# MarkTakken/kf2vecFSW

Measured on AMD Instinct MI355X. Metric: Gbases/s k-mer→.kf build at k=7; achieved HBM GB/s vs gfx950 peak, higher is better.
Workload: dtype u32

## Files before the change

### include/kf2vec_gpu.h

```cpp
#ifndef KF2VEC_GPU_H
#define KF2VEC_GPU_H

#include <stddef.h>
#include <stdint.h>

#ifdef __cplusplus
extern "C" {
#endif

#define KF_ABI_VERSION 1

#define KF_OK 0
#define KF_EINVAL (-1)
#define KF_EHIP (-2)
#define KF_ERANGE (-3)
#define KF_EFORMAT (-4)

#define KF_MIN_K 2
#define KF_MAX_K 12
#define KF_SPARSE_MAX_K 31

#define KF_ACCUMULATE 1u

#define KF_FMT_AUTO 0
// ... 19 lines not shown
int kf_index_fasta(const uint8_t* d_bytes, const uint64_t* d_goff, int32_t n_genomes,
                   uint64_t batch_bytes, uint64_t* d_excl, uint64_t cap_pairs,
                   uint64_t* d_n_pairs, uint32_t* d_scratch, uint64_t scratch_words, void* stream);

uint64_t kf_index_fastq_scratch_bytes(uint64_t batch_bytes, int32_t n_genomes, uint64_t cap_lines);
int kf_index_fastq(const uint8_t* d_bytes, const uint64_t* d_goff, int32_t n_genomes,
                   uint64_t batch_bytes, uint64_t* d_excl, uint64_t cap_pairs, uint64_t cap_lines,
                   uint64_t* d_n, uint32_t* d_status, void* d_scratch, uint64_t scratch_bytes,
                   void* stream);

int kf_count_batch(const uint8_t* d_bytes, const uint64_t* d_goff, int32_t n_genomes,
                   const uint64_t* d_excl, uint64_t n_excl,
                   const uint32_t* d_code2col, const uint32_t* d_col2rep, int k,
                   uint32_t* d_counts, uint64_t* d_totals, uint32_t flags, void* stream);

int kf_rows_accumulate(const uint32_t* d_src, const uint64_t* d_src_totals, int32_t n_src,
                       const int32_t* d_seg, int32_t n_dst, uint64_t nbins,
                       uint32_t* d_dst, uint64_t* d_dst_totals, uint32_t* d_status,
                       uint32_t flags, void* stream);

int kf_workspace_reserve(int k, int32_t max_genomes);

int kf_count_launch_info(int k, int* grid, int* block, int* lds_bytes);

uint64_t kf_sparse_workspace_bytes(int k, uint64_t batch_bytes, int32_t n_genomes);
int kf_sparse_count(const uint8_t* d_bytes, const uint64_t* d_goff, int32_t n_genomes,
                    uint64_t batch_bytes, const uint64_t* d_excl, uint64_t n_excl, int k,
                    void* d_work, uint64_t work_bytes, uint64_t* d_keys, uint32_t* d_counts,
                    uint64_t* d_nuniq, void* stream);

int kf_kmers_tile_rows(void);
int kf_kmers_rows(const uint64_t* d_keys, const void* d_counts, int count_bytes,
                  const uint64_t* d_src0, const uint64_t* d_n, const uint64_t* d_dst0,
                  const float* d_denom, int32_t n_seg, int k, uint64_t row_lo, uint64_t row_hi,
                  float* d_out, uint32_t* d_status, void* stream);

int      kf_sparse_merge_tile(void);
uint64_t kf_sparse_merge_scratch_bytes(uint64_t n_a, uint64_t n_b);
int kf_sparse_merge(const uint64_t* d_keys_a, const void* d_counts_a, int count_bytes_a, uint64_t n_a,
                    const uint64_t* d_keys_b, const void* d_counts_b, int count_bytes_b, uint64_t n_b,
                    uint64_t* d_keys_out, uint64_t* d_counts_out, uint64_t* d_n_out,
                    uint32_t* d_status, void* d_scratch, uint64_t scratch_bytes, void* stream);

uint64_t kf_chunk_features_scratch_bytes(int32_t n_samples);
int kf_chunk_features(const void* d_counts, int count_bytes, uint64_t n_rows, uint64_t nbins,
                      const uint64_t* d_lo, const uint64_t* d_n, int32_t n_samples,
// ... 59 lines not shown
```

### kf2vecfsw_amd/_native.py

```python
from __future__ import annotations

import ctypes
import os

_HERE = os.path.dirname(os.path.abspath(__file__))
LIB_PATH = os.environ.get("KF2VEC_GPU_LIB") or os.path.join(_HERE, "libkf2vec_gpu.so")

KF_OK = 0
KF_EINVAL = -1
KF_EHIP = -2
KF_ERANGE = -3
KF_EFORMAT = -4
KF_MIN_K = 2
KF_MAX_K = 12
KF_SPARSE_MAX_K = 31
KF_ACCUMULATE = 1
KF_FMT_AUTO, KF_FMT_FASTA, KF_FMT_FASTQ = 0, 1, 2

_u64, _u32, _i32, _i64, _int = ctypes.c_uint64, ctypes.c_uint32, ctypes.c_int32, ctypes.c_int64, ctypes.c_int
_vp, _cp = ctypes.c_void_p, ctypes.c_char_p
_P64 = ctypes.POINTER(ctypes.c_uint64)
_PI = ctypes.POINTER(ctypes.c_int)
SIGNATURES = {
    "kf_abi_version": (_int, []),
    "kf_last_error": (_cp, []),
    "kf_num_bins": (_u64, [_int]),
    "kf_tables": (_int, [_int, _vp, _vp, _P64]),
    "kf_vocab_text": (_int, [_int, _vp, _u64, _P64]),
    "kf_index_records": (_int, [_vp, _u64, _int, _u64, _vp, _u64, _P64, _PI]),
    "kf_count_batch": (_int, [_vp, _vp, _i32, _vp, _u64, _vp, _vp, _int, _vp, _vp, _u32, _vp]),
    "kf_rows_accumulate": (_int, [_vp, _vp, _i32, _vp, _i32, _u64, _vp, _vp, _vp, _u32, _vp]),
    "kf_count_launch_info": (_int, [_int, _PI, _PI, _PI]),
    "kf_workspace_release": (_int, []),
    "kf_workspace_reserve": (_int, [_int, _i32]),
    "kf_build_id": (_cp, []),
    "kf_stream_probe": (_int, [_vp, _u64, _vp, _vp]),
    "kf_synth_fasta": (_int, [_vp, _vp, _i32, _i64, _i64, _u64, _u64, _int, _u64, _vp]),
    "kf_synth_genome_bytes": (_u64, [_i64, _u64, _int, _u64]),
    "kf_synth_header_len": (_u64, [_i64]),
    "kf_format_kf": (_int, [_cp, _vp, _u64, _int, _int, _vp, _u64, _P64]),
    "kf_write_kf_files": (_int, [_cp, ctypes.POINTER(_cp), _i32, _vp, _u64, _int, _int, _int]),
    "kf_write_kf_rows": (_int, [_cp, ctypes.POINTER(_cp), _i32, _vp, _u64, _int, _int, _int]),
    "kf_write_kf_segments": (_int, [_i32, ctypes.POINTER(_cp), _vp, _vp, ctypes.POINTER(_cp), ctypes.POINTER(_cp),
                                    _vp, _vp, _u32, _vp, _u64, _int, _int, _int]),
    "kf_write_kf_segments16": (_int, [_i32, ctypes.POINTER(_cp), _vp, _vp, ctypes.POINTER(_cp), ctypes.POINTER(_cp),
                                      _vp, _vp, _u32, _vp, _u64, _int, _int, _int]),
    "kf_chunk_compact": (_int, [_vp, _u64, _vp, _i32, _vp, _vp, _vp, _u64, _vp]),
    "kf_chunk_gather": (_int, [_vp, _vp, _i32, _u32, _vp, _vp]),
    "kf_index_fasta": (_int, [_vp, _vp, _i32, _u64, _vp, _u64, _vp, _vp, _u64, _vp]),
    "kf_index_fastq_scratch_bytes": (_u64, [_u64, _i32, _u64]),
    "kf_index_fastq": (_int, [_vp, _vp, _i32, _u64, _vp, _u64, _u64, _vp, _vp, _vp, _u64, _vp]),
    "kf_read_files":(_int, [ctypes.POINTER(_cp), _i32, _vp, _vp, _vp, _u64, _int]),
    "kf_sparse_workspace_bytes": (_u64, [_int, _u64, _i32]),
    "kf_sparse_count": (_int, [_vp, _vp, _i32, _u64, _vp, _u64, _int, _vp, _u64, _vp, _vp, _vp, _vp]),
    "kf_kmers_tile_rows": (_int, []),
# ... 6 lines not shown
                                 _vp]),
    "kf_parse_kf_scratch_bytes": (_u64, [_u64, _i32, _u64]),
    "kf_parse_kf_rows": (_int, [_vp, _vp, _i32, _u64, _u64, _u64, _vp, _vp, _vp, _vp, _u64, _vp]),
}


class NativeError(RuntimeError):
    pass


_lib = None


def lib() -> ctypes.CDLL:
    global _lib
    if _lib is None:
        if not os.path.exists(LIB_PATH):
            raise NativeError(f"{LIB_PATH} not found: build it with `python -m kf2vecfsw_amd.build`")
        import torch
        try:
            L = ctypes.CDLL(LIB_PATH)
        except OSError as e:
            raise NativeError(f"cannot load {LIB_PATH}: {e}") from e
        for name, (res, args) in SIGNATURES.items():
            fn = getattr(L, name)
            fn.restype = res
            fn.argtypes = args
        if L.kf_abi_version() != 1:
            raise NativeError("libkf2vec_gpu ABI version mismatch")
        bid = L.kf_build_id().decode()
        if "+" not in bid and os.environ.get("KF2VEC_ALLOW_FOREIGN_LIB") != "1":
            from .build import source_id
            if bid != source_id():
                raise NativeError(f"{LIB_PATH} was built from other sources (build id {bid}, sources "
                                  f"{source_id()}): rebuild with `python -m kf2vecfsw_amd.build`")
        _lib = L
    return _lib


def build_id() -> str:
    return lib().kf_build_id().decode()


def check(rc: int, what: str = "") -> None:
    if rc != KF_OK:
        msg = lib().kf_last_error().decode(errors="replace")
        raise NativeError(f"{what or 'kf2vec_gpu'} failed ({rc}): {msg}")
```

### kf2vecfsw_amd/csrc/kf_bucket.hip

```cpp
#include <hip/hip_runtime.h>
#include <stdint.h>
#include <stdlib.h>

#include <algorithm>
#include <cstdio>
#include <mutex>
#include <vector>

#include "kf_front.h"
#include "kf_internal.h"

namespace kf {


constexpr int kBkWaves = 16;
constexpr int kBkBits = 15;
constexpr uint64_t kPieceMax = (8ull << 20) - (64ull << 10);
constexpr uint32_t kBkLagShift = 3;
constexpr uint32_t kBkSlots = 2;
constexpr uint32_t kBkRoundWeights = 0x060B1114;
constexpr int kBkGroupWindows = 4;
constexpr bool bk_pre2(int K) { return K <= 10; }
constexpr uint32_t bk_rl(int K) { return K == 10 ? 4 : 0; }

// ... 880 lines not shown
}

}

extern "C" int kf_workspace_release(void) {
    int dev = 0;
    if (hipGetDevice(&dev) != hipSuccess) return kf_fail(KF_EHIP, "hipGetDevice failed");
    if (dev < 0 || dev >= 64) return kf_fail(KF_EINVAL, "device index out of range");
    std::lock_guard<std::mutex> lk(g_mu);
    DevState& d = g_dev[dev];
    if (hipDeviceSynchronize() != hipSuccess) return kf_fail(KF_EHIP, "hipDeviceSynchronize failed");
    for (int k = 0; k <= KF_MAX_K; ++k) {
        if (d.col_idx[k]) (void)hipFree(d.col_idx[k]);
        if (d.bcol[k]) (void)hipFree(d.bcol[k]);
        d.col_idx[k] = nullptr;
        d.bcol[k] = nullptr;
    }
    if (d.scratch) (void)hipFree(d.scratch);
    if (d.pstart) (void)hipFree(d.pstart);
    d.scratch = nullptr;
    d.scratch_bytes = 0;
    d.pstart = nullptr;
    d.pstart_n = 0;
    return KF_OK;
}
```

### kf2vecfsw_amd/csrc/kf_count.hip

```cpp
#include <hip/hip_runtime.h>
#include <stdint.h>
#include <stdlib.h>

#include <mutex>

#include "kf_front.h"
#include "kf_internal.h"

namespace kf {

constexpr int kBlock = 1024;
constexpr uint32_t kWaveWeights = 20u | 17u << 8 | 11u << 16 | 6u << 24;
constexpr int kXRing = 2;

__device__ __forceinline__ void wg_span(const CountArgs& A, uint64_t& lo, uint64_t& hi) {
    const uint64_t base = A.goff[0];
    const uint64_t total = A.goff[A.n_genomes] - base;
    const uint64_t G = gridDim.x, b = blockIdx.x;
    lo = base + ((total / G * b + (total % G) * b / G) & ~(uint64_t)15);
    hi = (b + 1 == G) ? base + total : base + ((total / G * (b + 1) + (total % G) * (b + 1) / G) & ~(uint64_t)15);
}

template <int K>
struct XL {
    static constexpr uint32_t P = K >= 8 ? (1u << 17) : (2u << (2 * (K + 1)));
    static constexpr uint32_t S = K >= 8 ? (1u << 15) : (2u << (2 * K));
    static constexpr uint32_t bytes = P + S;
};
constexpr int kXChunk = 3 * kChunk;
static_assert((uint32_t)kXChunk == kLattice, "wave ranges are split on the iteration lattice (split_at_lattice)");
constexpr uint32_t kLatticeMaxIters = 2560;
constexpr uint32_t kHot7 = 0xC000C000u, kStep7 = 0x4000u;
constexpr uint32_t kHot8 = 0xE000E000u, kStep8 = 0x2000u;
constexpr uint32_t kHot6 = 0x80008000u, kStep6 = 0x8000u;
template <int K>
constexpr uint32_t x_hot() { return K >= 8 ? kHot8 : (K == 7 ? kHot7 : kHot6); }
template <int K>
constexpr uint32_t x_step() { return K >= 8 ? kStep8 : (K == 7 ? kStep7 : kStep6); }

__device__ __forceinline__ uint32_t k9_code_of(uint32_t i) { return ((i >> 9) << 10) | (i & 0x1FFu); }

__device__ __forceinline__ uint32_t half_one(uint32_t i) { return 1u << ((i & 1u) << 4); }

template <int B>
__device__ __forceinline__ uint32_t shl1_byte(uint32_t h, uint32_t one) {
    uint32_t r;
    if constexpr (B == 0)
        asm("v_lshlrev_b32_sdwa %0, %1, %2 dst_sel:DWORD dst_unused:UNUSED_PAD src0_sel:BYTE_0 src1_sel:DWORD"
            : "=v"(r) : "v"(h), "v"(one));
    else if constexpr (B == 1)
        asm("v_lshlrev_b32_sdwa %0, %1, %2 dst_sel:DWORD dst_unused:UNUSED_PAD src0_sel:BYTE_1 src1_sel:DWORD"
// ... 302 lines not shown
    if constexpr (K == 9) {
        drained |= k9b_region<false>(wlo, whi, R, A, gcounts);
        lane_total += (uint32_t)__builtin_popcount(R);
        return win.next;
    }
    const uint32_t wv[4] = {wlo, __builtin_amdgcn_alignbit(whi, wlo, 8), __builtin_amdgcn_alignbit(whi, wlo, 16),
                            __builtin_amdgcn_alignbit(whi, wlo, 24)};
    uint32_t o = 0;
#pragma unroll
    for (int r = 0; r < 16; ++r) {
        const int fo = (2 * r) & ~7;
        const uint32_t y = __builtin_amdgcn_ubfe(wv[fo >> 3], 2 * r - fo, 2 * K);
        o |= lds_add_rtn((K == 8 ? 0u : XL<K>::P) + ((y >> 1) << 2), ((R >> r) & 1u) * half_one(y));
    }
    if (__builtin_amdgcn_ballot_w64((o & HOT) != 0) != 0) {
        x_scan_drain<K>(A.code2col, gcounts, lane);
        drained = 1;
    }
    lane_total += (uint32_t)__builtin_popcount(R);
    return win.next;
}

template <int K>
__device__ __forceinline__ uint32_t x_range(const CountArgs& A, int32_t g, uint64_t glo, uint64_t ghi, uint64_t lo,
                                            uint64_t hi, int lane, uint64_t& iv_hint, uint32_t& drained) {
    if (lo >= hi) return 0;
    uint32_t* gcounts = A.counts + (uint64_t)g * A.nbins;
    Range rg;
    rg.init(glo, ghi, lo, hi);
    const uint32_t lim_r = min(rg.end_r, rg.nch * (uint32_t)kChunk);
    auto load = [&](uint32_t r) {
        return xc_load(A.bytes, rg.c0, r, lim_r, lane);
    };
    static_assert(kXRing == 2, "two-deep register ring");
    XBlock buf[K == 9 ? 1 : kXRing];
    XBlock b0, b1;
    if constexpr (K == 9) {
        b0 = load(0);
        b1 = load(kXChunk);
    } else {
#pragma unroll
        for (int j = 0; j < kXRing; ++j) buf[j] = load(j * kXChunk);
    }
    const uint32_t nx = (rg.nch + 2) / 3;
    rg.warm16<K>(A, lane, iv_hint);
    __builtin_amdgcn_s_setprio(0);
    uint32_t carry = rg.carry;
    uint32_t rel = 0;
    const ChunkMask m = rg.mask();
    uint32_t lane_total = 0;
// ... 71 lines not shown
__device__ __forceinline__ void pair_f_sums_small(const uint32_t* hist, int tid,
                                                  uint32_t (&F)[((1u << (2 * K)) + kBlock - 1) / kBlock]) {
    constexpr uint32_t NY = 1u << (2 * K), NM = (NY + kBlock - 1) / kBlock;
#pragma unroll
    for (uint32_t m = 0; m < NM; ++m) {
        const uint32_t y = (uint32_t)tid + kBlock * m;
        F[m] = 0;
        if (y < NY) {
            const uint32_t sh = (y & 1u) << 4;
            uint32_t f = u16sum2(hist[2 * y]) + u16sum2(hist[2 * y + 1]);
#pragma unroll
            for (uint32_t a = 0; a < 4; ++a) f += (hist[a * (NY / 2) + (y >> 1)] >> sh) & 0xFFFFu;
            f += (hist[XL<K>::P / 4 + (y >> 1)] >> sh) & 0xFFFFu;
            F[m] = f;
        }
    }
}

__device__ __forceinline__ void lds_zero(uint32_t* hist, uint32_t lo4, uint32_t hi4, int tid) {
    uint4* h4 = (uint4*)hist;
    for (uint32_t i = lo4 + (uint32_t)tid; i < hi4; i += kBlock) h4[i] = make_uint4(0u, 0u, 0u, 0u);
}

template <int K>
__global__ void __launch_bounds__(kBlock) __attribute__((amdgpu_waves_per_eu(4, 4))) k1x_kernel(CountArgs A) {
    static_assert(K >= 2 && K <= 9, "K1x serves k = 2 .. 9 (k = 9: K9b byte counters)");
    extern __shared__ __attribute__((aligned(16))) uint32_t hist[];
    const int tid = threadIdx.x;
    const int lane = tid & (kWave - 1);
    const int wave = __builtin_amdgcn_readfirstlane(tid >> 6);
    {
        uint4* h4 = (uint4*)hist;
        for (uint32_t i = tid; i < XL<K>::bytes / 16; i += kBlock) h4[i] = make_uint4(0u, 0u, 0u, 0u);
    }
    __syncthreads();
    if ((uint32_t)(uintptr_t)(lds_u32*)hist != 0u) __builtin_trap();
    uint64_t span_lo, span_hi;
    wg_span(A, span_lo, span_hi);
    if (span_lo >= span_hi) return;
    int32_t g = (int32_t)wave_upper_bound((uint64_t)A.n_genomes, span_lo, lane,
                                          [&](uint64_t i) { return A.goff[i + 1]; });
    const uint32_t fr_lo = wave_frac((uint32_t)wave, kWaveWeights), fr_hi = wave_frac((uint32_t)wave + 1, kWaveWeights);
    uint64_t g_lo = A.goff[g], g_hi = A.goff[g + 1];
    uint64_t iv_hint = 0;
    for (; g < A.n_genomes; ++g) {
        __builtin_amdgcn_s_setprio(3);
        const uint64_t glo = g_lo, ghi = g_hi;
        g_lo = g_hi;
        g_hi = A.goff[min(g + 2, A.n_genomes)];
        if (glo >= span_hi) break;
        const uint64_t plo = max(glo, span_lo), phi = min(ghi, span_hi);
        if (phi <= plo) continue;
        const uint32_t nit = lattice_iters(plo, phi);
        const bool lat = nit <= kLatticeMaxIters;
        const uint64_t lo = split_at_lattice(plo, phi, nit, lat, fr_lo), hi = split_at_lattice(plo, phi, nit, lat, fr_hi);
        uint32_t drained = 0;
        unsigned long long s = x_range<K>(A, g, glo, ghi, lo, hi, lane, iv_hint, drained);
        uint32_t* gc = A.counts + (uint64_t)g * A.nbins;
        const bool whole = plo == glo && phi == ghi && !(A.flags & KF_ACCUMULATE);
        if constexpr (K == 9) {
            lds_barrier();
            if (lane == 0) hist[XL<K>::P / 4 + wave] = drained;
            lds_barrier();
            const uint4* fl = (const uint4*)(hist + XL<K>::P / 4);
            const uint4 f0 = fl[0], f1 = fl[1], f2 = fl[2], f3 = fl[3];
            const bool any_fix = (f0.x | f0.y | f0.z | f0.w | f1.x | f1.y | f1.z | f1.w | f2.x | f2.y | f2.z |
                                  f2.w | f3.x | f3.y | f3.z | f3.w) != 0;
            const uint8_t* hb = (const uint8_t*)hist;
            for (uint32_t c0 = (uint32_t)tid; c0 < (1u << 17); c0 += 4 * kBlock) {
                uint32_t rep[4];
#pragma unroll
                for (int j = 0; j < 4; ++j) rep[j] = A.col2rep[c0 + j * kBlock];
#pragma unroll
                for (int j = 0; j < 4; ++j) {
                    const uint32_t c = (rep[j] & 0x200u) ? kf_revcomp<9>(rep[j]) : rep[j];
                    const uint32_t v = hb[((c >> 1) & 0x1FE00u) | (c & 0x1FFu)];
                    if (whole && !any_fix)
                        __builtin_nontemporal_store(v, gc + c0 + j * kBlock);
                    else if (v)
                        __hip_atomic_fetch_add(gc + c0 + j * kBlock, v, __ATOMIC_RELAXED, __HIP_MEMORY_SCOPE_AGENT);
                }
            }
            lds_barrier();
            uint4* h4 = (uint4*)hist;
            for (uint32_t i = tid; i < XL<K>::bytes / 16; i += kBlock) h4[i] = make_uint4(0u, 0u, 0u, 0u);
        } else if constexpr (K == 8) {
            lds_barrier();
            if (lane == 0) hist[XL<K>::P / 4 + wave] = drained;
            lds_barrier();
            const uint4* fl = (const uint4*)(hist + XL<K>::P / 4);
            const uint4 f0 = fl[0], f1 = fl[1], f2 = fl[2], f3 = fl[3];
            const bool any_drain = (f0.x | f0.y | f0.z | f0.w | f1.x | f1.y | f1.z | f1.w | f2.x | f2.y | f2.z |
                                    f2.w | f3.x | f3.y | f3.z | f3.w) != 0;
            for (uint32_t col = tid; col < A.nbins; col += kBlock) {
                const uint32_t y = A.col2rep[col], rc = kf_revcomp<8>(y);
                uint32_t v = (hist[y >> 1] >> ((y & 1u) << 4)) & 0xFFFFu;
                if (rc != y) v += (hist[rc >> 1] >> ((rc & 1u) << 4)) & 0xFFFFu;
                if (whole && !any_drain)
                    gc[col] = v;
                else if (v)
                    __hip_atomic_fetch_add(gc + col, v, __ATOMIC_RELAXED, __HIP_MEMORY_SCOPE_AGENT);
            }
            lds_barrier();
            uint4* h4 = (uint4*)hist;
            for (uint32_t i = tid; i < XL<K>::bytes / 16; i += kBlock) h4[i] = make_uint4(0u, 0u, 0u, 0u);
        } else if constexpr (K <= 6) {
            constexpr uint32_t NY = 1u << (2 * K), NM = (NY + kBlock - 1) / kBlock;
            constexpr uint32_t NCOL = (NY + (K % 2 == 0 ? (1u << K) : 0u)) / 2, NC = (NCOL + kBlock - 1) / kBlock;
            constexpr uint32_t ZF = (NY + 16) / 4;
            static_assert(ZF <= XL<K>::bytes / 16, "F and the flags lie inside the table");
            uint32_t rep[NC];
#pragma unroll
            for (uint32_t c = 0; c < NC; ++c) {
                const uint32_t col = (uint32_t)tid + c * kBlock;
                rep[c] = col < NCOL ? A.col2rep[col] : 0u;
            }
            lds_barrier();
            uint32_t F[NM];
            pair_f_sums_small<K>(hist, tid, F);
            lds_barrier();
#pragma unroll
            for (uint32_t m = 0; m < NM; ++m) {
                const uint32_t y = (uint32_t)tid + kBlock * m;
                if (y < NY) hist[f_swz(y)] = F[m];
            }
            if (lane == 0) hist[NY + wave] = drained;
            lds_zero(hist, ZF, XL<K>::bytes / 16, tid);
            lds_barrier();
            const uint4* fl = (const uint4*)(hist + NY);
            const uint4 f0 = fl[0], f1 = fl[1], f2 = fl[2], f3 = fl[3];
            const bool any_drain = (f0.x | f0.y | f0.z | f0.w | f1.x | f1.y | f1.z | f1.w | f2.x | f2.y | f2.z | f2.w |
                                    f3.x | f3.y | f3.z | f3.w) != 0;
            uint32_t cv[NC];
#pragma unroll
            for (uint32_t c = 0; c < NC; ++c) {
                const uint32_t y = rep[c], rc = kf_revcomp<K>(y);
                cv[c] = hist[f_swz(y)] + (rc != y ? hist[f_swz(rc)] : 0u);
            }
            lds_barrier();
            lds_zero(hist, 0, ZF, tid);
#pragma unroll
            for (uint32_t c = 0; c < NC; ++c) {
                const uint32_t col = (uint32_t)tid + c * kBlock;
                if (col >= NCOL) continue;
                if (whole && !any_drain)
                    __builtin_nontemporal_store(cv[c], gc + col);
                else if (cv[c])
                    __hip_atomic_fetch_add(gc + col, cv[c], __ATOMIC_RELAXED, __HIP_MEMORY_SCOPE_AGENT);
            }
        } else {
            uint32_t rep[8];
            if (whole) {
                const uint4 r0 = *(const uint4*)(A.col2rep + 4 * tid), r1 = *(const uint4*)(A.col2rep + 4096 + 4 * tid);
                rep[0] = r0.x, rep[1] = r0.y, rep[2] = r0.z, rep[3] = r0.w;
                rep[4] = r1.x, rep[5] = r1.y, rep[6] = r1.z, rep[7] = r1.w;
            } else {
#pragma unroll
                for (int c = 0; c < 8; ++c) rep[c] = A.col2rep[tid + c * kBlock];
            }
            lds_barrier();
            uint32_t F[16];
            pair_f_sums(hist, tid, F);
#pragma unroll
            for (int i = 0; i < 8; ++i) {
                const uint32_t v = hist[XL<K>::P / 4 + i * 1024 + tid];
                F[2 * i] += v & 0xFFFFu;
                F[2 * i + 1] += v >> 16;
            }
            lds_barrier();
#pragma unroll
            for (int i = 0; i < 8; ++i) *(uint2*)(hist + f_swz(i * 2048 + 2 * tid)) = make_uint2(F[2 * i], F[2 * i + 1]);
            if (lane == 0) hist[16384 + wave] = drained;
            constexpr uint32_t ZF = (16384 + 16) / 4;
            lds_zero(hist, ZF, XL<K>::bytes / 16, tid);
            lds_barrier();
            const uint4* fl = (const uint4*)(hist + 16384);
            const uint4 f0 = fl[0], f1 = fl[1], f2 = fl[2], f3 = fl[3];
            const bool any_drain = (f0.x | f0.y | f0.z | f0.w | f1.x | f1.y | f1.z | f1.w | f2.x | f2.y | f2.z | f2.w |
                                    f3.x | f3.y | f3.z | f3.w) != 0;
            uint32_t cv[8];
#pragma unroll
            for (int c = 0; c < 8; ++c) {
                const uint32_t y = rep[c], rc = kf_revcomp<7>(y);
                cv[c] = hist[f_swz(y)] + hist[f_swz(rc)];
            }
            lds_barrier();
            lds_zero(hist, 0, ZF, tid);
            if (whole && !any_drain) {
                typedef unsigned int v4u_t __attribute__((ext_vector_type(4)));
                __builtin_nontemporal_store(v4u_t{cv[0], cv[1], cv[2], cv[3]}, (v4u_t*)(gc + 4 * tid));
                __builtin_nontemporal_store(v4u_t{cv[4], cv[5], cv[6], cv[7]}, (v4u_t*)(gc + 4096 + 4 * tid));
            } else {
#pragma unroll
                for (int c = 0; c < 8; ++c) {
                    const uint32_t col = whole ? (c >> 2) * 4096 + 4 * tid + (c & 3) : tid + c * kBlock;
                    if (cv[c]) __hip_atomic_fetch_add(gc + col, cv[c], __ATOMIC_RELAXED, __HIP_MEMORY_SCOPE_AGENT);
                }
            }
        }
        s = wave_sum(s);
        if (lane == 0 && s) atomicAdd(A.totals + g, s);
        lds_barrier();
    }
}

__device__ __forceinline__ uint64_t splitmix64(uint64_t x) {
    x += 0x9E3779B97F4A7C15ull;
    x = (x ^ (x >> 30)) * 0xBF58476D1CE4E5B9ull;
    x = (x ^ (x >> 27)) * 0x94D049BB133111EBull;
    return x ^ (x >> 31);
}

__device__ __forceinline__ bool in_nrun(uint64_t key, uint64_t i, uint64_t n_period) {
    if (!n_period) return false;
    uint64_t b = i >> 12;
    for (int d = 0; d < 2; ++d) {
        if (d == 1) {
            if (b == 0) break;
            b -= 1;
        }
        const uint64_t h = splitmix64((key ^ 0xA5A5A5A5A5A5A5A5ull) + b);
        if (h % n_period) continue;
        const uint64_t st = (b << 12) + ((h >> 16) % 4096), ln = 1 + ((h >> 32) % 100);
        if (i >= st && i < st + ln) return true;
// ... 124 lines not shown
int launch_info(int k, int* grid, int* block, int* lds) {
    int dev = 0;
    if (hipGetDevice(&dev) != hipSuccess) return kf_fail(KF_EHIP, "hipGetDevice failed");
    if (dev < 0 || dev >= 64) return kf_fail(KF_EINVAL, "device index out of range");
    const int l = lds_bytes_for(k);
    std::lock_guard<std::mutex> lk(g_grid_mu);
    int& gr = g_grid[k][dev];
    if (!gr) {
        void* fn = kernel_for(k);
        if (hipFuncSetAttribute(fn, hipFuncAttributeMaxDynamicSharedMemorySize, l) != hipSuccess)
            return kf_fail(KF_EHIP, "hipFuncSetAttribute(MaxDynamicSharedMemorySize) failed");
        int per_cu = 0, cus = 0;
        if (hipOccupancyMaxActiveBlocksPerMultiprocessor(&per_cu, fn, kBlock, l) != hipSuccess)
            return kf_fail(KF_EHIP, "hipOccupancyMaxActiveBlocksPerMultiprocessor failed");
        if (hipDeviceGetAttribute(&cus, hipDeviceAttributeMultiprocessorCount, dev) != hipSuccess)
            return kf_fail(KF_EHIP, "hipDeviceGetAttribute(MultiprocessorCount) failed");
        gr = (per_cu < 1 ? 1 : per_cu) * (cus > 0 ? cus : 1);
    }
    *grid = gr;
    *block = kBlock;
    *lds = l;
    return KF_OK;
}
}

extern "C" int kf_count_launch_info(int k, int* grid, int* block, int* lds_bytes) {
    if (k < KF_MIN_K || k > KF_MAX_K) return kf_fail(KF_EINVAL, "k out of range [2, 12]");
    if (!grid || !block || !lds_bytes) return kf_fail(KF_EINVAL, "null output pointer");
    if (k >= 10) return bucket_launch_info(k, grid, block, lds_bytes);
    return launch_info(k, grid, block, lds_bytes);
}

extern "C" int kf_workspace_reserve(int k, int32_t max_genomes) {
    if (k < KF_MIN_K || k > KF_MAX_K) return kf_fail(KF_EINVAL, "k out of range [2, 12]");
    if (max_genomes < 0) return kf_fail(KF_EINVAL, "max_genomes < 0");
    if (k >= 10) return bucket_reserve(k, max_genomes);
    int grid = 0, block = 0, lds = 0;
    return launch_info(k, &grid, &block, &lds);
}

extern "C" int kf_count_batch(const uint8_t* d_bytes, const uint64_t* d_goff, int32_t n_genomes,
                              const uint64_t* d_excl, uint64_t n_excl, const uint32_t* d_code2col,
                              const uint32_t* d_col2rep, int k, uint32_t* d_counts, uint64_t* d_totals,
                              uint32_t flags, void* stream) {
    if (k < KF_MIN_K || k > KF_MAX_K) return kf_fail(KF_EINVAL, "k out of range [2, 12]");
    if (n_genomes < 0) return kf_fail(KF_EINVAL, "n_genomes < 0");
    if (n_genomes == 0) return KF_OK;
    if (!d_bytes || !d_goff || !d_counts || !d_totals || !d_code2col || !d_col2rep)
        return kf_fail(KF_EINVAL, "null device pointer");
    if (n_excl && !d_excl) return kf_fail(KF_EINVAL, "d_excl is null but n_excl > 0");
    if (((uintptr_t)d_bytes) & 15) return kf_fail(KF_EINVAL, "d_bytes must be 16-byte aligned");
    const uint64_t nb = kf_num_bins(k);
    hipStream_t s = (hipStream_t)stream;
    const bool bucket = k >= 10;
    if (!(flags & KF_ACCUMULATE)) {
        if ((!bucket && hipMemsetAsync(d_counts, 0, (size_t)n_genomes * nb * sizeof(uint32_t), s) != hipSuccess) ||
            hipMemsetAsync(d_totals, 0, (size_t)n_genomes * sizeof(uint64_t), s) != hipSuccess)
            return kf_fail(KF_EHIP, "hipMemsetAsync failed");
    }
    CountArgs A;
    A.bytes = d_bytes;
    A.goff = d_goff;
    A.excl = d_excl;
    A.n_excl = n_excl;
    A.code2col = d_code2col;
    A.col2rep = d_col2rep;
    A.counts = d_counts;
    A.totals = (unsigned long long*)d_totals;
    A.nbins = (uint32_t)nb;
    A.n_genomes = n_genomes;
    A.flags = flags;
    if (bucket) return bucket_launch(A, k, flags, s);
    int grid = 0, block = 0, lds = 0;
    const int rc = launch_info(k, &grid, &block, &lds);
    if (rc) return rc;

    void* args[] = {&A};
    if (hipLaunchKernel(kernel_for(k), dim3(grid), dim3(block), args, (size_t)lds, s) != hipSuccess)
        return kf_fail(KF_EHIP, "count kernel launch failed: %s", hipGetErrorString(hipGetLastError()));
    return KF_OK;
}

extern "C" int kf_stream_probe(const uint8_t* d_bytes, uint64_t n, uint32_t* d_out, void* stream) {
    if (!d_bytes || !d_out) return kf_fail(KF_EINVAL, "null device pointer");
    if (((uintptr_t)d_bytes) & 15) return kf_fail(KF_EINVAL, "d_bytes must be 16-byte aligned");
    if (n == 0) return KF_OK;
    int dev = 0, cus = 0;
    if (hipGetDevice(&dev) != hipSuccess ||
        hipDeviceGetAttribute(&cus, hipDeviceAttributeMultiprocessorCount, dev) != hipSuccess)
        return kf_fail(KF_EHIP, "device query failed");
    hipLaunchKernelGGL(stream_probe_kernel, dim3(2 * (cus > 0 ? cus : 1)), dim3(1024), 0, (hipStream_t)stream, d_bytes,
                       n, d_out);
    if (hipGetLastError() != hipSuccess) return kf_fail(KF_EHIP, "stream probe launch failed");
    return KF_OK;
}

extern "C" int kf_synth_fasta(uint8_t* d_bytes, const uint64_t* d_goff, int32_t n_genomes, int64_t g0,
                              int64_t g_stride, uint64_t seed0, uint64_t seq_len, int width, uint64_t n_period,
                              void* stream) {
// ... 11 lines not shown
```

### kf2vecfsw_amd/csrc/kf_front.h

```cpp
#pragma once
#include <hip/hip_runtime.h>
#include <stdint.h>

#include "kf_scan.h"

namespace kf {

constexpr int kWave = 64;
constexpr int kChunk = 1024;

struct CountArgs {
    const uint8_t* bytes;
    const uint64_t* goff;
    const uint64_t* excl;
    uint64_t n_excl;
    const uint32_t* code2col;
    const uint32_t* col2rep;
    uint32_t* counts;
    unsigned long long* totals;
    uint32_t nbins;
    int32_t n_genomes;
    uint32_t flags;
};

// ... 419 lines not shown
    }
    const uint64_t W = ((uint64_t)t_codes(ctx) << (2 * ne)) | (uint64_t)C;
    Windows w;
    w.wlo = (uint32_t)W;
    w.whi = (uint32_t)(W >> 32);
    const uint32_t ctxlen = min(t_n(ctx), (uint32_t)(K - 1));
    const uint32_t E = (((1u << ctxlen) - 1u) << ne) | V;
    w.R = run_mask<K>(E) & ((1u << ne) - 1u);
    if (MASKED) w.R &= EN;
    const uint32_t incl = tail_pack(w.wlo & TM, (uint32_t)__builtin_ctz(~E), 31u);
    w.next = (uint32_t)__builtin_amdgcn_readlane((int)incl, kWave - 1);
    return w;
}

__device__ __forceinline__ unsigned long long wave_sum(unsigned long long v) {
#pragma unroll
    for (int d = 32; d >= 1; d >>= 1) v += __shfl_xor(v, d, kWave);
    return v;
}

int bucket_launch(const CountArgs& A, int k, uint32_t flags, hipStream_t s);
int bucket_launch_info(int k, int* grid, int* block, int* lds);
int bucket_reserve(int k, int32_t max_genomes);

}
```

Baseline: 6058.

## Drop count-matrix memset via per-block scratch slots and last-arriver row finalize

Removes the host-side hipMemsetAsync of the full counts and totals arrays for k<10 non-accumulating batches. Whole genomes are written directly, empty genomes are zeroed in-kernel, and split genomes accumulate atomically into pre-zeroed per-owner workspace slots. The last block to arrive, detected with an arrival counter, copies the slot to the output row and re-zeroes it. This saves a full write pass over the count matrix, at the cost of a persistent workspace, cross-block atomics, extra LDS words and per-stream event ordering.

```diff
diff --git a/include/kf2vec_gpu.h b/include/kf2vec_gpu.h
--- a/include/kf2vec_gpu.h
+++ b/include/kf2vec_gpu.h
@@ -65,6 +65,9 @@
 int kf_workspace_reserve(int k, int32_t max_genomes);
 
 int kf_count_launch_info(int k, int* grid, int* block, int* lds_bytes);
+
+int kf_span_cuts(uint64_t total, uint32_t grid, uint64_t* cuts);
+int kf_span_owners(uint64_t total, uint32_t grid, const uint64_t* pos, uint64_t n, uint32_t* owner);
 
 uint64_t kf_sparse_workspace_bytes(int k, uint64_t batch_bytes, int32_t n_genomes);
 int kf_sparse_count(const uint8_t* d_bytes, const uint64_t* d_goff, int32_t n_genomes,
diff --git a/kf2vecfsw_amd/_native.py b/kf2vecfsw_amd/_native.py
--- a/kf2vecfsw_amd/_native.py
+++ b/kf2vecfsw_amd/_native.py
@@ -31,6 +31,8 @@
     "kf_count_batch": (_int, [_vp, _vp, _i32, _vp, _u64, _vp, _vp, _int, _vp, _vp, _u32, _vp]),
     "kf_rows_accumulate": (_int, [_vp, _vp, _i32, _vp, _i32, _u64, _vp, _vp, _vp, _u32, _vp]),
     "kf_count_launch_info": (_int, [_int, _PI, _PI, _PI]),
+    "kf_span_cuts": (_int, [_u64, _u32, _vp]),
+    "kf_span_owners": (_int, [_u64, _u32, _vp, _u64, _vp]),
     "kf_workspace_release": (_int, []),
     "kf_workspace_reserve": (_int, [_int, _i32]),
     "kf_build_id": (_cp, []),
@@ -83,8 +85,14 @@
             L = ctypes.CDLL(LIB_PATH)
         except OSError as e:
             raise NativeError(f"cannot load {LIB_PATH}: {e}") from e
+        foreign = os.environ.get("KF2VEC_ALLOW_FOREIGN_LIB") == "1"
         for name, (res, args) in SIGNATURES.items():
-            fn = getattr(L, name)
+            try:
+                fn = getattr(L, name)
+            except AttributeError as e:
+                if foreign:
+                    continue
+                raise NativeError(f"{LIB_PATH} lacks {name}: rebuild with `python -m kf2vecfsw_amd.build`") from e
             fn.restype = res
             fn.argtypes = args
         if L.kf_abi_version() != 1:
diff --git a/kf2vecfsw_amd/csrc/kf_bucket.hip b/kf2vecfsw_amd/csrc/kf_bucket.hip
--- a/kf2vecfsw_amd/csrc/kf_bucket.hip
+++ b/kf2vecfsw_amd/csrc/kf_bucket.hip
@@ -926,5 +926,5 @@
     d.scratch_bytes = 0;
     d.pstart = nullptr;
     d.pstart_n = 0;
-    return KF_OK;
-}
+    return count_workspace_release(dev);
+}
diff --git a/kf2vecfsw_amd/csrc/kf_count.hip b/kf2vecfsw_amd/csrc/kf_count.hip
--- a/kf2vecfsw_amd/csrc/kf_count.hip
+++ b/kf2vecfsw_amd/csrc/kf_count.hip
@@ -12,21 +12,41 @@
 constexpr int kBlock = 1024;
 constexpr uint32_t kWaveWeights = 20u | 17u << 8 | 11u << 16 | 6u << 24;
 constexpr int kXRing = 2;
+
+struct CountArgsX : CountArgs {
+    uint32_t* ws_slots;
+    unsigned long long* ws_arrived;
+    uint32_t slot_words;
+};
+
+__host__ __device__ inline uint64_t span_cut(uint64_t total, uint64_t G, uint64_t b) {
+    return b >= G ? total : (total / G * b + (total % G) * b / G) & ~(uint64_t)15;
+}
+__host__ __device__ inline uint32_t span_owner(uint64_t total, uint32_t G, uint64_t pos) {
+    uint32_t a = 0, b = G;
+    while (b - a > 1) {
+        const uint32_t m = a + (b - a) / 2;
+        if (span_cut(total, G, m) <= pos) a = m;
+        else b = m;
+    }
+    return a;
+}
 
 __device__ __forceinline__ void wg_span(const CountArgs& A, uint64_t& lo, uint64_t& hi) {
     const uint64_t base = A.goff[0];
     const uint64_t total = A.goff[A.n_genomes] - base;
     const uint64_t G = gridDim.x, b = blockIdx.x;
-    lo = base + ((total / G * b + (total % G) * b / G) & ~(uint64_t)15);
-    hi = (b + 1 == G) ? base + total : base + ((total / G * (b + 1) + (total % G) * (b + 1) / G) & ~(uint64_t)15);
+    lo = base + span_cut(total, G, b);
+    hi = base + span_cut(total, G, b + 1);
 }
 
 template <int K>
 struct XL {
     static constexpr uint32_t P = K >= 8 ? (1u << 17) : (2u << (2 * (K + 1)));
     static constexpr uint32_t S = K >= 8 ? (1u << 15) : (2u << (2 * K));
-    static constexpr uint32_t bytes = P + S;
+    static constexpr uint32_t bytes = (K <= 6 && P + S < 4u * ((1u << (2 * K)) + 48u)) ? 4u * ((1u << (2 * K)) + 48u) : P + S;
 };
+constexpr uint32_t kFlushWords = 48;
 constexpr int kXChunk = 3 * kChunk;
 static_assert((uint32_t)kXChunk == kLattice, "wave ranges are split on the iteration lattice (split_at_lattice)");
 constexpr uint32_t kLatticeMaxIters = 2560;
@@ -375,10 +395,9 @@
 }
 
 template <int K>
-__device__ __forceinline__ uint32_t x_range(const CountArgs& A, int32_t g, uint64_t glo, uint64_t ghi, uint64_t lo,
-                                            uint64_t hi, int lane, uint64_t& iv_hint, uint32_t& drained) {
+__device__ __forceinline__ uint32_t x_range(const CountArgs& A, uint32_t* gcounts, uint64_t glo, uint64_t ghi,
+                                            uint64_t lo, uint64_t hi, int lane, uint64_t& iv_hint, uint32_t& drained) {
     if (lo >= hi) return 0;
-    uint32_t* gcounts = A.counts + (uint64_t)g * A.nbins;
     Range rg;
     rg.init(glo, ghi, lo, hi);
     const uint32_t lim_r = min(rg.end_r, rg.nch * (uint32_t)kChunk);
@@ -496,19 +515,143 @@
     for (uint32_t i = lo4 + (uint32_t)tid; i < hi4; i += kBlock) h4[i] = make_uint4(0u, 0u, 0u, 0u);
 }
 
+struct PieceOut {
+    uint32_t* row;
+    uint32_t* add;
+    unsigned long long* total;
+    unsigned long long* add_total;
+    unsigned long long* arrived;
+    bool whole;
+};
+
+__device__ __forceinline__ void slot_sync() {
+    asm volatile("s_waitcnt vmcnt(0)" ::: "memory");
+    __syncthreads();
+}
+__device__ __forceinline__ uint32_t slot_load(const uint32_t* p) {
+    return __hip_atomic_load(p, __ATOMIC_RELAXED, __HIP_MEMORY_SCOPE_AGENT);
+}
+__device__ __forceinline__ void slot_zero(uint32_t* p) {
+    __hip_atomic_store(p, 0u, __ATOMIC_RELAXED, __HIP_MEMORY_SCOPE_AGENT);
+}
+__device__ __forceinline__ void row_put(const PieceOut& o, uint32_t col, uint32_t v) {
+    asm volatile("" : "+v"(col));
+    const uint32_t d = slot_load(o.add + col);
+    o.row[col] = v + d;
+    if (d) slot_zero(o.add + col);
+}
+__device__ __forceinline__ void put_wave_words(uint32_t* hist, uint32_t f, int wave, int lane, uint32_t drained,
+                                               unsigned long long s) {
+    if (lane == 0) {
+        hist[f + wave] = drained;
+        *(uint2*)(hist + f + 16 + 2 * wave) = make_uint2((uint32_t)s, (uint32_t)(s >> 32));
+    }
+}
+__device__ __forceinline__ void put_whole_total(const uint32_t* hist, uint32_t f, int tid, bool whole,
+                                                unsigned long long* total) {
+    if (whole && tid == 0) {
+        const uint4* w = (const uint4*)(hist + f + 16);
+        unsigned long long t = 0;
+#pragma unroll
+        for (int i = 0; i < 8; ++i) {
+            const uint4 v = w[i];
+            t += ((unsigned long long)v.y << 32 | v.x) + ((unsigned long long)v.w << 32 | v.z);
+        }
+        *total = t;
+    }
+}
+
+__device__ __forceinline__ void piece_finish(const PieceOut& o, uint32_t* hist, int tid, int lane, unsigned long long s,
+                                             uint64_t piece, uint64_t genome, uint32_t nbins) {
+    if (lane == 0 && s) atomicAdd(o.add_total, s);
+    if (!o.arrived) return;
+    slot_sync();
+    if (tid == 0) {
+        const unsigned long long old = __hip_atomic_fetch_add(o.arrived, (unsigned long long)piece, __ATOMIC_RELAXED,
+                                                              __HIP_MEMORY_SCOPE_AGENT);
+        hist[0] = old + piece == genome ? 1u : 0u;
+    }
+    __syncthreads();
+    const bool last = hist[0] != 0u;
+    __syncthreads();
+    if (tid == 0) hist[0] = 0u;
+    if (!last) return;
+    uint32_t col0 = (uint32_t)tid;
+    asm volatile("" : "+v"(col0));
+    if ((nbins & 3u) == 0 && ((uintptr_t)o.row & 15u) == 0) {
+        constexpr int kSc1 = 16;
+        typedef unsigned int v4u_t __attribute__((ext_vector_type(4)));
+        const auto rs = __builtin_amdgcn_make_buffer_rsrc((void*)o.add, (short)0, (int)(nbins * 4u), 0x00020000);
+        const uint32_t n4 = nbins / 4u;
+        for (uint32_t i0 = col0; i0 < n4; i0 += 8 * kBlock) {
+            v4u_t v[8];
+#pragma unroll
+            for (int j = 0; j < 8; ++j)
+                v[j] = __builtin_amdgcn_raw_buffer_load_b128(rs, (int)((i0 + j * kBlock) * 16u), 0, kSc1);
+#pragma unroll
+            for (int j = 0; j < 8; ++j) {
+                const uint32_t i = i0 + j * kBlock;
+                if (i < n4) *(v4u_t*)(o.row + 4u * i) = v[j];
+                if (v[j][0] | v[j][1] | v[j][2] | v[j][3])
+                    __builtin_amdgcn_raw_buffer_store_b128(v4u_t{0u, 0u, 0u, 0u}, rs, (int)(i * 16u), 0, kSc1);
+            }
+        }
+    } else
+    for (uint32_t c0 = col0; c0 < nbins; c0 += 8 * kBlock) {
+        uint32_t v[8];
+#pragma unroll
+        for (int j = 0; j < 8; ++j) v[j] = c0 + j * kBlock < nbins ? slot_load(o.add + c0 + j * kBlock) : 0u;
+#pragma unroll
+        for (int j = 0; j < 8; ++j) {
+            const uint32_t col = c0 + j * kBlock;
+            if (col < nbins) o.row[col] = v[j];
+            if (v[j]) slot_zero(o.add + col);
+        }
+    }
+    if (tid == 0) {
+        *o.total = __hip_atomic_load(o.add_total, __ATOMIC_RELAXED, __HIP_MEMORY_SCOPE_AGENT);
+        __hip_atomic_store(o.add_total, 0ull, __ATOMIC_RELAXED, __HIP_MEMORY_SCOPE_AGENT);
+        __hip_atomic_store(o.arrived, 0ull, __ATOMIC_RELAXED, __HIP_MEMORY_SCOPE_AGENT);
+    }
+}
+
+__device__ __forceinline__ void zero_empty_rows(const CountArgs& A, int tid, int lane, uint64_t e_lo, uint64_t e_hi) {
+    const uint64_t n = (uint64_t)A.n_genomes, stride = (uint64_t)gridDim.x * kBlock;
+    for (uint64_t g0 = (uint64_t)blockIdx.x * kBlock; g0 < n; g0 += stride) {
+        uint64_t m = __ballot(e_lo == e_hi);
+        while (m) {
+            const uint64_t ge = g0 + (uint64_t)(tid & ~(kWave - 1)) + (uint64_t)__builtin_ctzll(m);
+            m &= m - 1;
+            uint32_t* r = A.counts + ge * A.nbins;
+            for (uint32_t c = (uint32_t)lane; c < A.nbins; c += kWave) r[c] = 0u;
+            if (lane == 0) A.totals[ge] = 0ull;
+        }
+        const uint64_t gi = g0 + stride + (uint64_t)tid;
+        e_lo = ~0ull, e_hi = 0;
+        if (gi < n) e_lo = A.goff[gi], e_hi = A.goff[gi + 1];
+    }
+}
+
 template <int K>
-__global__ void __launch_bounds__(kBlock) __attribute__((amdgpu_waves_per_eu(4, 4))) k1x_kernel(CountArgs A) {
+__global__ void __launch_bounds__(kBlock) __attribute__((amdgpu_waves_per_eu(4, 4))) k1x_kernel(CountArgsX A) {
     static_assert(K >= 2 && K <= 9, "K1x serves k = 2 .. 9 (k = 9: K9b byte counters)");
     extern __shared__ __attribute__((aligned(16))) uint32_t hist[];
     const int tid = threadIdx.x;
     const int lane = tid & (kWave - 1);
     const int wave = __builtin_amdgcn_readfirstlane(tid >> 6);
+    const bool acc = (A.flags & KF_ACCUMULATE) != 0;
+    uint64_t e_lo = ~0ull, e_hi = 0;
+    if (!acc) {
+        const uint64_t gi = (uint64_t)blockIdx.x * kBlock + (uint64_t)tid;
+        if (gi < (uint64_t)A.n_genomes) e_lo = A.goff[gi], e_hi = A.goff[gi + 1];
+    }
     {
         uint4* h4 = (uint4*)hist;
         for (uint32_t i = tid; i < XL<K>::bytes / 16; i += kBlock) h4[i] = make_uint4(0u, 0u, 0u, 0u);
     }
     __syncthreads();
     if ((uint32_t)(uintptr_t)(lds_u32*)hist != 0u) __builtin_trap();
+    if (!acc) zero_empty_rows(A, tid, lane, e_lo, e_hi);
     uint64_t span_lo, span_hi;
     wg_span(A, span_lo, span_hi);
     if (span_lo >= span_hi) return;
@@ -529,17 +672,38 @@
         const bool lat = nit <= kLatticeMaxIters;
         const uint64_t lo = split_at_lattice(plo, phi, nit, lat, fr_lo), hi = split_at_lattice(plo, phi, nit, lat, fr_hi);
         uint32_t drained = 0;
-        unsigned long long s = x_range<K>(A, g, glo, ghi, lo, hi, lane, iv_hint, drained);
-        uint32_t* gc = A.counts + (uint64_t)g * A.nbins;
-        const bool whole = plo == glo && phi == ghi && !(A.flags & KF_ACCUMULATE);
+        uint32_t slot = 2u * blockIdx.x;
+        if (!acc && !(plo == glo && phi == ghi)) {
+            uint32_t owner = blockIdx.x;
+            if (plo != glo) {
+                const uint64_t base = A.goff[0];
+                owner = span_owner(A.goff[A.n_genomes] - base, gridDim.x, glo - base);
+            }
+            slot = 2u * owner + 1u;
+        }
+        uint32_t* const gc = acc ? A.counts + (uint64_t)g * A.nbins : A.ws_slots + (uint64_t)slot * A.slot_words;
+        const unsigned long long s = wave_sum(x_range<K>(A, gc, glo, ghi, lo, hi, lane, iv_hint, drained));
+        const bool whole = plo == glo && phi == ghi && !acc;
+        PieceOut out;
+        out.whole = whole;
+        out.row = A.counts + (uint64_t)g * A.nbins;
+        out.add = gc;
+        out.total = out.add_total = A.totals + g;
+        out.arrived = nullptr;
+        if (!acc && !whole) {
+            out.add_total = (unsigned long long*)(gc + (A.slot_words - 4u));
+            out.arrived = A.ws_arrived + (slot >> 1);
+        }
         if constexpr (K == 9) {
             lds_barrier();
-            if (lane == 0) hist[XL<K>::P / 4 + wave] = drained;
+            put_wave_words(hist, XL<K>::P / 4, wave, lane, drained, s);
             lds_barrier();
             const uint4* fl = (const uint4*)(hist + XL<K>::P / 4);
             const uint4 f0 = fl[0], f1 = fl[1], f2 = fl[2], f3 = fl[3];
             const bool any_fix = (f0.x | f0.y | f0.z | f0.w | f1.x | f1.y | f1.z | f1.w | f2.x | f2.y | f2.z |
                                   f2.w | f3.x | f3.y | f3.z | f3.w) != 0;
+            put_whole_total(hist, XL<K>::P / 4, tid, whole, out.total);
+            if (whole && any_fix) slot_sync();
             const uint8_t* hb = (const uint8_t*)hist;
             for (uint32_t c0 = (uint32_t)tid; c0 < (1u << 17); c0 += 4 * kBlock) {
                 uint32_t rep[4];
@@ -550,39 +714,47 @@
                     const uint32_t c = (rep[j] & 0x200u) ? kf_revcomp<9>(rep[j]) : rep[j];
                     const uint32_t v = hb[((c >> 1) & 0x1FE00u) | (c & 0x1FFu)];
                     if (whole && !any_fix)
-                        __builtin_nontemporal_store(v, gc + c0 + j * kBlock);
+                        __builtin_nontemporal_store(v, out.row + c0 + j * kBlock);
+                    else if (whole)
+                        row_put(out, c0 + j * kBlock, v);
                     else if (v)
                         __hip_atomic_fetch_add(gc + c0 + j * kBlock, v, __ATOMIC_RELAXED, __HIP_MEMORY_SCOPE_AGENT);
                 }
             }
+            if (whole && any_fix) slot_sync();
             lds_barrier();
             uint4* h4 = (uint4*)hist;
             for (uint32_t i = tid; i < XL<K>::bytes / 16; i += kBlock) h4[i] = make_uint4(0u, 0u, 0u, 0u);
         } else if constexpr (K == 8) {
             lds_barrier();
-            if (lane == 0) hist[XL<K>::P / 4 + wave] = drained;
+            put_wave_words(hist, XL<K>::P / 4, wave, lane, drained, s);
             lds_barrier();
             const uint4* fl = (const uint4*)(hist + XL<K>::P / 4);
             const uint4 f0 = fl[0], f1 = fl[1], f2 = fl[2], f3 = fl[3];
             const bool any_drain = (f0.x | f0.y | f0.z | f0.w | f1.x | f1.y | f1.z | f1.w | f2.x | f2.y | f2.z |
                                     f2.w | f3.x | f3.y | f3.z | f3.w) != 0;
+            put_whole_total(hist, XL<K>::P / 4, tid, whole, out.total);
+            if (whole && any_drain) slot_sync();
             for (uint32_t col = tid; col < A.nbins; col += kBlock) {
                 const uint32_t y = A.col2rep[col], rc = kf_revcomp<8>(y);
                 uint32_t v = (hist[y >> 1] >> ((y & 1u) << 4)) & 0xFFFFu;
                 if (rc != y) v += (hist[rc >> 1] >> ((rc & 1u) << 4)) & 0xFFFFu;
                 if (whole && !any_drain)
-                    gc[col] = v;
+                    out.row[col] = v;
+                else if (whole)
+                    row_put(out, col, v);
                 else if (v)
                     __hip_atomic_fetch_add(gc + col, v, __ATOMIC_RELAXED, __HIP_MEMORY_SCOPE_AGENT);
             }
+            if (whole && any_drain) slot_sync();
             lds_barrier();
             uint4* h4 = (uint4*)hist;
             for (uint32_t i = tid; i < XL<K>::bytes / 16; i += kBlock) h4[i] = make_uint4(0u, 0u, 0u, 0u);
         } else if constexpr (K <= 6) {
             constexpr uint32_t NY = 1u << (2 * K), NM = (NY + kBlock - 1) / kBlock;
             constexpr uint32_t NCOL = (NY + (K % 2 == 0 ? (1u << K) : 0u)) / 2, NC = (NCOL + kBlock - 1) / kBlock;
-            constexpr uint32_t ZF = (NY + 16) / 4;
-            static_assert(ZF <= XL<K>::bytes / 16, "F and the flags lie inside the table");
+            constexpr uint32_t ZF = (NY + kFlushWords) / 4;
+            static_assert(ZF <= XL<K>::bytes / 16, "F and the per-wave words lie inside the table");
             uint32_t rep[NC];
 #pragma unroll
             for (uint32_t c = 0; c < NC; ++c) {
@@ -598,7 +770,7 @@
                 const uint32_t y = (uint32_t)tid + kBlock * m;
                 if (y < NY) hist[f_swz(y)] = F[m];
             }
-            if (lane == 0) hist[NY + wave] = drained;
+            put_wave_words(hist, NY, wave, lane, drained, s);
             lds_zero(hist, ZF, XL<K>::bytes / 16, tid);
             lds_barrier();
             const uint4* fl = (const uint4*)(hist + NY);
@@ -611,17 +783,22 @@
                 const uint32_t y = rep[c], rc = kf_revcomp<K>(y);
                 cv[c] = hist[f_swz(y)] + (rc != y ? hist[f_swz(rc)] : 0u);
             }
+            put_whole_total(hist, NY, tid, whole, out.total);
             lds_barrier();
             lds_zero(hist, 0, ZF, tid);
+            if (whole && any_drain) slot_sync();
 #pragma unroll
             for (uint32_t c = 0; c < NC; ++c) {
                 const uint32_t col = (uint32_t)tid + c * kBlock;
                 if (col >= NCOL) continue;
                 if (whole && !any_drain)
-                    __builtin_nontemporal_store(cv[c], gc + col);
+                    __builtin_nontemporal_store(cv[c], out.row + col);
+                else if (whole)
+                    row_put(out, col, cv[c]);
                 else if (cv[c])
                     __hip_atomic_fetch_add(gc + col, cv[c], __ATOMIC_RELAXED, __HIP_MEMORY_SCOPE_AGENT);
             }
+            if (whole && any_drain) slot_sync();
         } else {
             uint32_t rep[8];
             if (whole) {
@@ -644,8 +821,8 @@
             lds_barrier();
 #pragma unroll
             for (int i = 0; i < 8; ++i) *(uint2*)(hist + f_swz(i * 2048 + 2 * tid)) = make_uint2(F[2 * i], F[2 * i + 1]);
-            if (lane == 0) hist[16384 + wave] = drained;
-            constexpr uint32_t ZF = (16384 + 16) / 4;
+            put_wave_words(hist, 16384, wave, lane, drained, s);
+            constexpr uint32_t ZF = (16384 + kFlushWords) / 4;
             lds_zero(hist, ZF, XL<K>::bytes / 16, tid);
             lds_barrier();
             const uint4* fl = (const uint4*)(hist + 16384);
@@ -658,22 +835,25 @@
                 const uint32_t y = rep[c], rc = kf_revcomp<7>(y);
                 cv[c] = hist[f_swz(y)] + hist[f_swz(rc)];
             }
+            put_whole_total(hist, 16384, tid, whole, out.total);
             lds_barrier();
             lds_zero(hist, 0, ZF, tid);
             if (whole && !any_drain) {
                 typedef unsigned int v4u_t __attribute__((ext_vector_type(4)));
-                __builtin_nontemporal_store(v4u_t{cv[0], cv[1], cv[2], cv[3]}, (v4u_t*)(gc + 4 * tid));
-                __builtin_nontemporal_store(v4u_t{cv[4], cv[5], cv[6], cv[7]}, (v4u_t*)(gc + 4096 + 4 * tid));
+                __builtin_nontemporal_store(v4u_t{cv[0], cv[1], cv[2], cv[3]}, (v4u_t*)(out.row + 4 * tid));
+                __builtin_nontemporal_store(v4u_t{cv[4], cv[5], cv[6], cv[7]}, (v4u_t*)(out.row + 4096 + 4 * tid));
+            } else if (whole) {
+                slot_sync();
+#pragma unroll
+                for (int c = 0; c < 8; ++c) row_put(out, (c >> 2) * 4096 + 4 * tid + (c & 3), cv[c]);
+                slot_sync();
             } else {
 #pragma unroll
-                for (int c = 0; c < 8; ++c) {
-                    const uint32_t col = whole ? (c >> 2) * 4096 + 4 * tid + (c & 3) : tid + c * kBlock;
-                    if (cv[c]) __hip_atomic_fetch_add(gc + col, cv[c], __ATOMIC_RELAXED, __HIP_MEMORY_SCOPE_AGENT);
-                }
-            }
-        }
-        s = wave_sum(s);
-        if (lane == 0 && s) atomicAdd(A.totals + g, s);
+                for (int c = 0; c < 8; ++c)
+                    if (cv[c]) __hip_atomic_fetch_add(gc + tid + c * kBlock, cv[c], __ATOMIC_RELAXED, __HIP_MEMORY_SCOPE_AGENT);
+            }
+        }
+        if (!whole) piece_finish(out, hist, tid, lane, s, phi - plo, ghi - glo, A.nbins);
         lds_barrier();
     }
 }
@@ -844,6 +1024,65 @@
     *lds = l;
     return KF_OK;
 }
+
+struct CountWs {
+    void* buf = nullptr;
+    size_t bytes = 0;
+    hipEvent_t ev = nullptr;
+    hipStream_t last = nullptr;
+    bool used = false;
+};
+CountWs g_ws[64];
+std::mutex g_ws_mu;
+
+uint32_t slot_words_for(int k) { return (((uint32_t)kf_num_bins(k) + 3u) & ~3u) + 4u; }
+
+int ensure_count_ws(CountWs& w, int k, int grid) {
+    const size_t need = (size_t)grid * (2 * (size_t)slot_words_for(k) * 4 + 8);
+    if (w.bytes >= need) return KF_OK;
+    if (!w.ev && hipEventCreateWithFlags(&w.ev, hipEventDisableTiming) != hipSuccess)
+        return kf_fail(KF_EHIP, "hipEventCreate failed");
+    if (hipDeviceSynchronize() != hipSuccess || (w.buf && hipFree(w.buf) != hipSuccess))
+        return kf_fail(KF_EHIP, "hipFree of the count workspace failed");
+    w.buf = nullptr;
+    w.bytes = 0;
+    w.used = false;
+    if (hipMalloc(&w.buf, need) != hipSuccess)
+        return kf_fail(KF_EHIP, "hipMalloc of %zu bytes of count workspace failed", need);
+    if (hipMemset(w.buf, 0, need) != hipSuccess || hipDeviceSynchronize() != hipSuccess) {
+        (void)hipFree(w.buf);
+        w.buf = nullptr;
+        return kf_fail(KF_EHIP, "zeroing the count workspace failed");
+    }
+    w.bytes = need;
+    return KF_OK;
+}
+}
+
+namespace kf {
+int count_workspace_release(int dev) {
+    std::lock_guard<std::mutex> lk(g_ws_mu);
+    CountWs& w = g_ws[dev];
+    if (w.buf) (void)hipFree(w.buf);
+    w.buf = nullptr;
+    w.bytes = 0;
+    w.used = false;
+    return KF_OK;
+}
+}
+
+extern "C" int kf_span_cuts(uint64_t total, uint32_t grid, uint64_t* cuts) {
+    if (!grid || !cuts) return kf_fail(KF_EINVAL, "kf_span_cuts: grid 0 or null cuts");
+    for (uint32_t b = 0; b <= grid; ++b) cuts[b] = span_cut(total, grid, b);
+    return KF_OK;
+}
+
+extern "C" int kf_span_owners(uint64_t total, uint32_t grid, const uint64_t* pos, uint64_t n, uint32_t* owner) {
+    if (!grid || (n && (!pos || !owner))) return kf_fail(KF_EINVAL, "kf_span_owners: grid 0 or null pointer");
+    for (uint64_t i = 0; i < n; ++i)
+        if (pos[i] >= total) return kf_fail(KF_EINVAL, "kf_span_owners: position %llu past the batch", (unsigned long long)pos[i]);
+    for (uint64_t i = 0; i < n; ++i) owner[i] = span_owner(total, grid, pos[i]);
+    return KF_OK;
 }
 
 extern "C" int kf_count_launch_info(int k, int* grid, int* block, int* lds_bytes) {
@@ -858,7 +1097,12 @@
     if (max_genomes < 0) return kf_fail(KF_EINVAL, "max_genomes < 0");
     if (k >= 10) return bucket_reserve(k, max_genomes);
     int grid = 0, block = 0, lds = 0;
-    return launch_info(k, &grid, &block, &lds);
+    const int rc = launch_info(k, &grid, &block, &lds);
+    if (rc) return rc;
+    int dev = 0;
+    if (hipGetDevice(&dev) != hipSuccess) return kf_fail(KF_EHIP, "hipGetDevice failed");
+    std::lock_guard<std::mutex> lk(g_ws_mu);
+    return ensure_count_ws(g_ws[dev], k, grid);
 }
 
 extern "C" int kf_count_batch(const uint8_t* d_bytes, const uint64_t* d_goff, int32_t n_genomes,
@@ -875,12 +1119,10 @@
     const uint64_t nb = kf_num_bins(k);
     hipStream_t s = (hipStream_t)stream;
     const bool bucket = k >= 10;
-    if (!(flags & KF_ACCUMULATE)) {
-        if ((!bucket && hipMemsetAsync(d_counts, 0, (size_t)n_genomes * nb * sizeof(uint32_t), s) != hipSuccess) ||
-            hipMemsetAsync(d_totals, 0, (size_t)n_genomes * sizeof(uint64_t), s) != hipSuccess)
-            return kf_fail(KF_EHIP, "hipMemsetAsync failed");
-    }
-    CountArgs A;
+    if (bucket && !(flags & KF_ACCUMULATE) &&
+        hipMemsetAsync(d_totals, 0, (size_t)n_genomes * sizeof(uint64_t), s) != hipSuccess)
+        return kf_fail(KF_EHIP, "hipMemsetAsync failed");
+    CountArgsX A;
     A.bytes = d_bytes;
     A.goff = d_goff;
     A.excl = d_excl;
@@ -894,9 +1136,31 @@
     A.flags = flags;
     if (bucket) return bucket_launch(A, k, flags, s);
     int grid = 0, block = 0, lds = 0;
-    const int rc = launch_info(k, &grid, &block, &lds);
+    int rc = launch_info(k, &grid, &block, &lds);
     if (rc) return rc;
-
+    int dev = 0;
+    if (hipGetDevice(&dev) != hipSuccess) return kf_fail(KF_EHIP, "hipGetDevice failed");
+    std::lock_guard<std::mutex> lk(g_ws_mu);
+    CountWs& w = g_ws[dev];
+    A.ws_slots = nullptr;
+    A.ws_arrived = nullptr;
+    A.slot_words = slot_words_for(k);
+    if (!(flags & KF_ACCUMULATE)) {
+        rc = ensure_count_ws(w, k, grid);
+        if (rc) return rc;
+        A.ws_slots = (uint32_t*)w.buf;
+        A.ws_arrived = (unsigned long long*)((char*)w.buf + (size_t)grid * 2 * A.slot_words * 4);
+        if (w.used && w.last != s) {
+            if (hipEventRecord(w.ev, w.last) != hipSuccess) {
+                (void)hipGetLastError();
+                if (hipDeviceSynchronize() != hipSuccess) return kf_fail(KF_EHIP, "hipDeviceSynchronize failed");
+            } else if (hipStreamWaitEvent(s, w.ev, 0) != hipSuccess) {
+                return kf_fail(KF_EHIP, "hipStreamWaitEvent failed");
+            }
+        }
+        w.last = s;
+        w.used = true;
+    }
     void* args[] = {&A};
     if (hipLaunchKernel(kernel_for(k), dim3(grid), dim3(block), args, (size_t)lds, s) != hipSuccess)
         return kf_fail(KF_EHIP, "count kernel launch failed: %s", hipGetErrorString(hipGetLastError()));
diff --git a/kf2vecfsw_amd/csrc/kf_front.h b/kf2vecfsw_amd/csrc/kf_front.h
--- a/kf2vecfsw_amd/csrc/kf_front.h
+++ b/kf2vecfsw_amd/csrc/kf_front.h
@@ -465,5 +465,6 @@
 int bucket_launch(const CountArgs& A, int k, uint32_t flags, hipStream_t s);
 int bucket_launch_info(int k, int* grid, int* block, int* lds);
 int bucket_reserve(int k, int32_t max_genomes);
-
-}
+int count_workspace_release(int dev);
+
+}
```

Result: no change. 6056 (-0.0%).
